# themattinthehatt/behavenet

Measured on AMD Instinct MI355X. Metric: AE training frames/sec (128x128x1, batch 256), higher is better.
Workload: dtype f32; 1 GPU; configs[1]: conv AE default arch, 1x128x128 f32 frames resident in HBM, 12 latents, batch 256 (chunks 200+56), fwd+bwd+Adam(amsgrad)

## Files before the change

### behavenet_amd/_hip.py

```python

import ctypes
import os

import torch

_LIB_NAME = 'libbehavenet_hip.so'
_LIB_PATH = os.environ.get('BN_HIP_LIB') or os.path.join(
    os.path.dirname(os.path.abspath(__file__)), _LIB_NAME)
_lib = None

ACT_NONE, ACT_LRELU, ACT_SIGMOID = 0, 1, 2

PROF_NONE, PROF_CONV_FWD, PROF_CONV_BWD_D, PROF_CONV_BWD_W = 0, 1, 2, 3
PROF_CONVT_FWD, PROF_CONVT_BWD_D, PROF_CONVT_BWD_W, PROF_ADAM = 4, 5, 6, 7
PROF_LINEAR_FWD, PROF_LINEAR_BWD = 8, 9

_c_int, _c_float, _c_size_t, _c_void_p = ctypes.c_int, ctypes.c_float, ctypes.c_size_t, ctypes.c_void_p

_CONV_GEOM = [_c_int] * 12
_ACT_WS = [_c_int, _c_float, _c_void_p, _c_size_t, _c_void_p]

OP_CONV_FWD, OP_CONV_BWD_D, OP_CONV_BWD_W = 1, 2, 3
OP_CONVT_FWD, OP_CONVT_BWD_D, OP_CONVT_BWD_W = 4, 5, 6

# ... 41 lines not shown
    'bn_conv2d_pool2_act_ok': (_c_int, _CONV_GEOM),
    'bn_conv2d_pool2_bwd_weight_ws_bytes': (_c_size_t, _CONV_GEOM),
    'bn_conv2d_pool2_bwd_weight': (
        _c_int, [_c_void_p] * 6 + _CONV_GEOM + [_c_int, _c_float, _c_int, _c_void_p, _c_size_t, _c_void_p]),
    'bn_maxpool2d_act_bwd': (_c_int, [_c_void_p] * 4 + [_c_int] * 4 + [ctypes.c_float, _c_void_p]),
    'bn_maxunpool2d_fwd': (_c_int, [_c_void_p] * 3 + [_c_int] * 3 + [_c_void_p]),
    'bn_maxunpool2d_fwd_k2': (_c_int, [_c_void_p] * 3 + [_c_int] * 3 + [_c_void_p]),
    'bn_maxunpool2d_bwd': (_c_int, [_c_void_p] * 3 + [_c_int] * 3 + [_c_void_p]),
    'bn_act_fwd': (_c_int, [_c_void_p] * 2 + [_c_size_t, _c_int, _c_float, _c_void_p]),
    'bn_act_bwd': (_c_int, [_c_void_p] * 3 + [_c_size_t, _c_int, _c_float, _c_void_p]),
    'bn_linear_ws_bytes': (_c_size_t, [_c_int] * 3),
    'bn_linear_fwd': (_c_int, [_c_void_p] * 4 + [_c_int] * 3 + [_c_void_p, _c_size_t, _c_void_p]),
    'bn_linear_bwd': (
        _c_int, [_c_void_p] * 5 + [_c_int, _c_float, _c_void_p, _c_void_p, _c_int] +
        [_c_int] * 3 + [_c_void_p, _c_size_t, _c_void_p]),
    'bn_sqerr_frame_sums': (_c_int, [_c_void_p] * 4 + [_c_int, _c_size_t, _c_void_p]),
    'bn_sqerr_bwd': (_c_int, [_c_void_p] * 4 + [_c_size_t, _c_float, _c_void_p, _c_void_p]),
    'bn_convT2d_fwd_sqerr_parts': (_c_int, _CONV_GEOM),
    'bn_convT2d_fwd_sqerr_ws_bytes': (_c_size_t, _CONV_GEOM + [_c_int]),
    'bn_convT2d_fwd_sqerr': (
        _c_int, [_c_void_p] * 8 + _CONV_GEOM + [_c_int, _c_float, _c_void_p, _c_size_t, _c_void_p]),
    'bn_scale_frames': (_c_int, [_c_void_p] * 4 + [_c_int, _c_size_t, _c_void_p]),
    'bn_reduce_sum': (_c_int, [_c_void_p] * 2 + [_c_size_t, _c_float, _c_void_p]),
    'bn_reparam_fwd': (_c_int, [_c_void_p] * 4 + [_c_size_t, _c_void_p]),
    'bn_kl_rows': (_c_int, [_c_void_p] * 3 + [_c_int, _c_int, _c_void_p]),
    'bn_reparam_bwd': (_c_int, [_c_void_p] * 4 + [_c_size_t, _c_void_p]),
    'bn_kl_bwd': (_c_int, [_c_void_p] * 4 + [_c_size_t, _c_float, _c_void_p, _c_void_p]),
    'bn_decomposed_kl_fwd': (_c_int, [_c_void_p] * 7 + [_c_int, _c_int, _c_void_p]),
    'bn_decomposed_kl_bwd': (_c_int, [_c_void_p] * 9 + [_c_int, _c_int, _c_void_p]),
    'bn_psvae_head_fwd': (_c_int, [_c_void_p] * 14 + [_c_int] * 3 + [_c_void_p]),
    'bn_psvae_head_combine': (
        _c_int, [_c_void_p] * 4 + [_c_int] + [_c_float] * 3 + [_c_int] + [_c_void_p] * 3),
    'bn_psvae_head_bwd': (
        _c_int, [_c_void_p] * 3 + [_c_int] + [_c_void_p] * 10 + [_c_float] + [_c_void_p] * 5 +
        [_c_int] * 4 + [_c_void_p]),
    'bn_adam_amsgrad_step': (
        _c_int, [_c_void_p] * 5 + [_c_size_t] + [_c_float] * 5 + [_c_int, _c_void_p]),
    'bn_conv2d_first_bf16_ok': (_c_int, _CONV_GEOM),
    'bn_conv2d_bf16_ok': (_c_int, _CONV_GEOM),
    'bn_conv_pack_w_bf16_bytes': (_c_size_t, [_c_int] * 4),
    'bn_conv_pack_w_bf16': (_c_int, [_c_void_p] * 2 + [_c_int] * 4 + [_c_void_p]),
    'bn_conv2d_first_bf16': (
        _c_int, [_c_void_p, _c_int] + [_c_void_p] * 3 + _CONV_GEOM + [_c_int, _c_float, _c_void_p]),
    'bn_conv2d_fwd_bf16': (
        _c_int, [_c_void_p] * 4 + [_c_int] + _CONV_GEOM + [_c_int, _c_float, _c_void_p]),
    'bn_convT2d_bf16_ok': (_c_int, _CONV_GEOM),
# ... 663 lines not shown
        _ptr(dpre, 'dpre'), _ptr(part, 'part'), *geom, act, slope, ws, nbytes, _stream()),
        'bn_convT2d_fwd_sqerr')
    return xhat, dpre, part


def scale_frames(t, frame_scale, group_scale=None, group_of_frame=None):
    N = t.shape[0]
    _check(load().bn_scale_frames(
        _ptr(t, 't'), _ptr(frame_scale, 'frame_scale'),
        _ptr(group_scale, 'group_scale', allow_none=True),
        _ptr(group_of_frame, 'group_of_frame', dtype=torch.int32, allow_none=True),
        N, t.numel() // N, _stream()), 'bn_scale_frames')
    return t


def reduce_sum(t, scale=1.0, out=None):
    if out is None:
        out = torch.empty((), dtype=torch.float32, device=t.device)
    _check(load().bn_reduce_sum(_ptr(t, 'in'), _ptr(out, 'out'), t.numel(), float(scale),
                                _stream()), 'bn_reduce_sum')
    return out


def reparam_fwd(mu, logvar, eps):
    z = torch.empty_like(mu)
    _check(load().bn_reparam_fwd(
        _ptr(mu, 'mu'), _ptr(logvar, 'logvar'), _ptr(eps, 'eps'), _ptr(z, 'z'), mu.numel(),
        _stream()), 'bn_reparam_fwd')
    return z


def kl_rows(mu, logvar):
    N, D = mu.shape
    out = torch.empty((N,), dtype=torch.float32, device=mu.device)
    _check(load().bn_kl_rows(_ptr(mu, 'mu'), _ptr(logvar, 'logvar'), _ptr(out, 'kl_rows'), N, D,
                             _stream()), 'bn_kl_rows')
    return out


DECOMPOSED_KL_MAX_D = 64


def _check_dkl_width(D):
    if D > DECOMPOSED_KL_MAX_D:
        raise ValueError('decomposed KL: %d latent dimensions, the kernels serve at most %d'
                         % (D, DECOMPOSED_KL_MAX_D))
# ... 233 lines not shown
```

### behavenet_amd/csrc/bn_launch.h

```cpp
#pragma once
#include "bn_common.h"

struct GemmArgs {
    const float* A; long sai, sak;
    const float* B; long sbk, sbj;
    float* C; long sci, scj;
    int M, N, K;
    const float* bias_j;
    const float* dact_src;
    int dact; float slope;
    int accumulate;
    float* part;
    int kslice;
};

int bn_launch_down_generic(const float* big, const float* w, const float* bias, float* out,
                           const float* dact_src, const BnGeom& g, int act, int dact, float slope,
                           hipStream_t st);
int bn_launch_up_generic(const float* small, const float* w, const float* bias, float* out,
                         const float* dact_src, const BnGeom& g, int act, int dact, float slope,
                         hipStream_t st);
int bn_launch_wgrad_generic(const float* small, const float* big, float* dw, const BnGeom& g,
                            int accumulate, hipStream_t st);
size_t bn_channel_sum_ws_bytes(int N, int C, int npix);
int bn_launch_channel_sum(const float* t, float* db, int N, int C, int npix, int accumulate,
                          void* ws, size_t ws_bytes, hipStream_t st);

int bn_launch_gemm(const GemmArgs& a, hipStream_t st, void* ws = nullptr, size_t ws_bytes = 0);
size_t bn_gemm_ws_bytes(int M, int N, int K);
int bn_launch_col_sum(const float* dy, float* db, int M, int N, int accumulate, hipStream_t st);
int bn_launch_linear_jobs(const GemmArgs* g0, const GemmArgs* g1, const float* dy, float* db, int M,
                          int N, int accumulate, void* ws, size_t ws_bytes, hipStream_t st);
size_t bn_linear_jobs_ws_bytes(int M, int N, int K);

int bn_launch_act_fwd(const float* x, float* y, size_t n, int act, float slope, hipStream_t st);
int bn_launch_act_bwd(const float* dy, const float* y, float* dpre, size_t n, int act, float slope,
                      hipStream_t st);
int bn_launch_sqerr_frame_sums(const float* pred, const float* target, const float* mask,
                               float* frame_sums, int N, size_t D, hipStream_t st);
int bn_launch_sqerr_bwd(const float* pred, const float* target, const float* mask, float* dpred,
                        size_t n, float scale, const float* gscale, hipStream_t st);
int bn_launch_scale_frames(float* t, const float* frame_scale, const float* group_scale,
                           const int* group_of_frame, int N, size_t D, hipStream_t st);
int bn_launch_reduce_sum(const float* in, float* out, size_t n, float scale, hipStream_t st);
int bn_launch_reparam_fwd(const float* mu, const float* logvar, const float* eps, float* z,
                          size_t n, hipStream_t st);
int bn_launch_kl_rows(const float* mu, const float* logvar, float* kl_rows, int N, int D,
                      hipStream_t st);
int bn_launch_reparam_bwd(const float* dz, const float* z, const float* mu, float* dlogvar,
                          size_t n, hipStream_t st);
int bn_launch_kl_bwd(const float* mu, const float* logvar, float* dmu, float* dlogvar, size_t n,
                     float scale, const float* gscale, hipStream_t st);
int bn_launch_adam(float* p, const float* g, float* m, float* v, float* vmax, size_t n, float lr,
                   float b1, float b2, float eps, float wd, int step, hipStream_t st);
int bn_launch_u8_to_unit_float(const unsigned char* in, float* out, size_t n, hipStream_t st);

bool bn_frame_sq_err_ok(int N, size_t D);
size_t bn_frame_sq_err_ws_bytes_impl(int N, size_t D);
int bn_launch_frame_sq_err(const float* xhat, const void* target, int target_is_u8, const float* mask, float* out,
                           int N, size_t D, float scale, void* ws, hipStream_t st);
int bn_launch_frame_err_finish(const float* part, float* out, int N, unsigned P, float scale, hipStream_t st);

bool bn_unit_float_to_u8_ok(size_t n);
int bn_launch_unit_float_to_u8(const float* in, unsigned char* out, size_t n, hipStream_t st);

size_t bn_batchnorm_ws_bytes_impl(int N, int C);
int bn_launch_bn_stats(const float* x, float* mean, float* var, int N, int C, int HW, void* ws,
// ... 114 lines not shown
```

### behavenet_amd/csrc/capi.hip

```cpp
#include <math.h>
#include <stdio.h>
#include <stdlib.h>
#include <string.h>
#include <hip/hip_ext.h>
#include "bn_common.h"
#include "bn_launch.h"
#include "bn_fast.h"

namespace {
struct ProfState {
    int family = BN_PROF_NONE;
    int C = 0, K = 0;
    static const int kMaxSlots = 2048;
    hipEvent_t ev[4 * kMaxSlots];
    bool taken[kMaxSlots], bracketed[kMaxSlots];
    int created = 0;
    int used = 0;
    double total_ms = 0.0, main_ms = 0.0;
    long launches = 0, main_launches = 0;
    bool bracket = true;
    int nth = -1, seen = 0;
    char kernel_name[96] = "";
} g_prof;

// ... 1554 lines not shown
    if (rc) return rc;
    rc = bn_launch_sqerr_frame_sums(xh, target, mask, part, N, (size_t)Co * Ho * Wo, st);
    if (rc) return rc;
    rc = bn_launch_sqerr_bwd(xh, target, mask, dpre, n_out, 1.f, nullptr, st);
    if (rc) return rc;
    if (act != BN_ACT_NONE) rc = bn_launch_act_bwd(dpre, xh, dpre, n_out, act, slope, st);
    return rc;
}

extern "C" int bn_scale_frames(float* t, const float* frame_scale, const float* group_scale,
                               const int* group_of_frame, int N, size_t D, bn_stream_t stream) {
    if (!t || !frame_scale || N <= 0 || D == 0) return BN_E_BADARG;
    if ((group_scale == nullptr) != (group_of_frame == nullptr)) return BN_E_BADARG;
    return bn_launch_scale_frames(t, frame_scale, group_scale, group_of_frame, N, D,
                                  (hipStream_t)stream);
}

extern "C" int bn_reduce_sum(const float* in, float* out, size_t n, float scale,
                             bn_stream_t stream) {
    if (!in || !out) return BN_E_BADARG;
    return bn_launch_reduce_sum(in, out, n, scale, (hipStream_t)stream);
}

extern "C" int bn_reparam_fwd(const float* mu, const float* logvar, const float* eps, float* z,
                              size_t n, bn_stream_t stream) {
    if (!mu || !logvar || !eps || !z) return BN_E_BADARG;
    if (n == 0) return 0;
    return bn_launch_reparam_fwd(mu, logvar, eps, z, n, (hipStream_t)stream);
}

extern "C" int bn_kl_rows(const float* mu, const float* logvar, float* kl_rows, int N, int D,
                          bn_stream_t stream) {
    if (!mu || !logvar || !kl_rows || N <= 0 || D <= 0) return BN_E_BADARG;
    return bn_launch_kl_rows(mu, logvar, kl_rows, N, D, (hipStream_t)stream);
}

extern "C" int bn_reparam_bwd(const float* dz, const float* z, const float* mu, float* dlogvar,
                              size_t n, bn_stream_t stream) {
    if (!dz || !z || !mu || !dlogvar) return BN_E_BADARG;
    if (n == 0) return 0;
    return bn_launch_reparam_bwd(dz, z, mu, dlogvar, n, (hipStream_t)stream);
}

extern "C" int bn_kl_bwd(const float* mu, const float* logvar, float* dmu, float* dlogvar,
                         size_t n, float scale, const float* gscale, bn_stream_t stream) {
    if (!mu || !logvar || !dmu || !dlogvar) return BN_E_BADARG;
// ... 200 lines not shown
```

### behavenet_amd/csrc/elementwise.hip

```cpp
#include "bn_common.h"
#include "bn_launch.h"

#define EW_THREADS 256
#define EW_MAX_BLOCKS 2048

static inline int ew_blocks(size_t nvec) {
    size_t b = (nvec + EW_THREADS - 1) / EW_THREADS;
    if (b < 1) b = 1;
    if (b > EW_MAX_BLOCKS) b = EW_MAX_BLOCKS;
    return (int)b;
}

static inline bool aligned16(const void* p) { return (((uintptr_t)p) & 15u) == 0; }

__global__ __launch_bounds__(EW_THREADS) void k_act_bwd(
    const float* __restrict__ dy, const float* __restrict__ y, float* __restrict__ dpre, size_t n,
    int vec, int act, float slope) {
    const size_t tid = (size_t)blockIdx.x * EW_THREADS + threadIdx.x;
    const size_t nthreads = (size_t)gridDim.x * EW_THREADS;
    if (vec) {
        const size_t n4 = n >> 2;
        const float4* dy4 = reinterpret_cast<const float4*>(dy);
        const float4* y4 = reinterpret_cast<const float4*>(y);
        float4* o4 = reinterpret_cast<float4*>(dpre);
// ... 71 lines not shown
            if (mask) { const float4 k = m4[i]; o.x *= k.x; o.y *= k.y; o.z *= k.z; o.w *= k.w; }
            o4[i] = o;
        }
        for (size_t i = (n4 << 2) + tid; i < n; i += nthreads) {
            float o = sc * (pred[i] - target[i]); if (mask) o *= mask[i]; dpred[i] = o;
        }
    } else {
        for (size_t i = tid; i < n; i += nthreads) {
            float o = sc * (pred[i] - target[i]); if (mask) o *= mask[i]; dpred[i] = o;
        }
    }
}

__global__ __launch_bounds__(EW_THREADS) void k_reduce_sum(
    const float* __restrict__ in, float* __restrict__ out, size_t n, float scale) {
    __shared__ float red[EW_THREADS / BN_WAVE];
    float acc = 0.f;
    for (size_t i = threadIdx.x; i < n; i += EW_THREADS) acc += in[i];
#pragma unroll
    for (int off = 32; off > 0; off >>= 1) acc += __shfl_down(acc, off, 64);
    if ((threadIdx.x & 63) == 0) red[threadIdx.x >> 6] = acc;
    __syncthreads();
    if (threadIdx.x == 0) out[0] = ((red[0] + red[1]) + (red[2] + red[3])) * scale;
}

__global__ __launch_bounds__(EW_THREADS) void k_reparam_fwd(
    const float* __restrict__ mu, const float* __restrict__ logvar, const float* __restrict__ eps,
    float* __restrict__ z, size_t n) {
    const size_t nthreads = (size_t)gridDim.x * EW_THREADS;
    for (size_t i = (size_t)blockIdx.x * EW_THREADS + threadIdx.x; i < n; i += nthreads)
        z[i] = fmaf(eps[i], expf(logvar[i]), mu[i]);
}

__global__ __launch_bounds__(EW_THREADS) void k_kl_rows(
    const float* __restrict__ mu, const float* __restrict__ logvar, float* __restrict__ kl_rows,
    int N, int D) {
    const int row = blockIdx.x * (EW_THREADS / BN_WAVE) + (threadIdx.x >> 6);
    if (row >= N) return;
    const int lane = threadIdx.x & 63;
    float acc = 0.f;
    for (int d = lane; d < D; d += BN_WAVE) {
        const float lv = logvar[(size_t)row * D + d], m = mu[(size_t)row * D + d];
        acc += expf(lv) - lv + m * m - 1.f;
    }
#pragma unroll
    for (int off = 32; off > 0; off >>= 1) acc += __shfl_down(acc, off, 64);
// ... 152 lines not shown
    } else {
        for (size_t i = tid; i < D; i += nthreads) row[i] *= sc;
    }
}

int bn_launch_scale_frames(float* t, const float* frame_scale, const float* group_scale,
                           const int* group_of_frame, int N, size_t D, hipStream_t st) {
    const int vec = aligned16(t) && (D % 4 == 0);
    const size_t per = vec ? D / 4 : D;
    int bx = (int)((per + EW_THREADS - 1) / EW_THREADS);
    if (bx > 64) bx = 64;
    hipLaunchKernelGGL(k_scale_frames, dim3(bx, N), dim3(EW_THREADS), 0, st, t, frame_scale,
                       group_scale, group_of_frame, D, vec);
    BN_LAUNCH_CHECK();
    return 0;
}

int bn_launch_reduce_sum(const float* in, float* out, size_t n, float scale, hipStream_t st) {
    hipLaunchKernelGGL(k_reduce_sum, dim3(1), dim3(EW_THREADS), 0, st, in, out, n, scale);
    BN_LAUNCH_CHECK();
    return 0;
}

int bn_launch_reparam_fwd(const float* mu, const float* logvar, const float* eps, float* z,
                          size_t n, hipStream_t st) {
    hipLaunchKernelGGL(k_reparam_fwd, dim3(ew_blocks(n)), dim3(EW_THREADS), 0, st, mu, logvar, eps,
                       z, n);
    BN_LAUNCH_CHECK();
    return 0;
}

int bn_launch_kl_rows(const float* mu, const float* logvar, float* kl_rows, int N, int D,
                      hipStream_t st) {
    const int rows_per_block = EW_THREADS / BN_WAVE;
    hipLaunchKernelGGL(k_kl_rows, dim3((N + rows_per_block - 1) / rows_per_block),
                       dim3(EW_THREADS), 0, st, mu, logvar, kl_rows, N, D);
    BN_LAUNCH_CHECK();
    return 0;
}

int bn_launch_reparam_bwd(const float* dz, const float* z, const float* mu, float* dlogvar,
                          size_t n, hipStream_t st) {
    hipLaunchKernelGGL(k_reparam_bwd, dim3(ew_blocks(n)), dim3(EW_THREADS), 0, st, dz, z, mu,
                       dlogvar, n);
    BN_LAUNCH_CHECK();
    return 0;
// ... 32 lines not shown
```

### behavenet_amd/hip_functions.py

```python

import collections.abc
import contextlib
import os
import threading
import warnings

import torch

from behavenet_amd import _hip

LRELU_SLOPE = 0.05

_direct_grads = False


class accumulate_into_param_grads(object):

    def __enter__(self):
        global _direct_grads
        self._prev = _direct_grads
        _direct_grads = True

    def __exit__(self, *exc):
        global _direct_grads
# ... 373 lines not shown
                    rec[i].append((acts[i + 1] > 0).cpu())
        ctx.plan = plan
        ctx.taps = taps
        ctx.need_dx = x.requires_grad
        ctx.param_refs = params
        _note_use(params, any(ctx.needs_input_grad[3:]))
        ctx.save_for_backward(*acts, *params[0::2])
        return h

    @staticmethod
    def backward(ctx, dout):
        plan = ctx.plan
        dout = dout.contiguous()
        top = plan[-1]
        if top.act != _hip.ACT_NONE:
            dpre = _hip.act_bwd(dout, ctx.saved_tensors[len(plan)], top.act, LRELU_SLOPE)
        else:
            dpre = dout
        dx, grads = _stack_backward(ctx, dpre, first_param=3)
        return (None, dx, None) + tuple(grads)


_DGRAD_FIRST = os.environ.get('BN_DGRAD_FIRST', '0') == '1'


def _stack_backward(ctx, dpre, first_param):
    plan = ctx.plan
    n_layers = len(plan)
    saved = ctx.saved_tensors
    acts, weights = saved[:n_layers + 1], saved[n_layers + 1:2 * n_layers + 1]
    n = dpre.shape[0]
    grads = [None] * (2 * n_layers)
    taps = getattr(ctx, 'taps', None)
    tail = []
    for i in range(n_layers - 1, -1, -1):
        layer = plan[i]
        g = layer.geom(n)
        w = weights[i]
        x_in = acts[i]
        if x_in.dtype == torch.uint8:
            x_in = _hip.u8_to_unit_float(x_in) \
                if ctx.needs_input_grad[first_param + 2 * i] else None
        need_w = ctx.needs_input_grad[first_param + 2 * i]
        need_b = ctx.needs_input_grad[first_param + 1 + 2 * i]
        dpre_below = None
        if i > 0 and min(plan[i - 1].cin, plan[i - 1].cout) <= 4 and _DGRAD_FIRST:
            dact_src, dact = acts[i], plan[i - 1].act
            bwd_data = _hip.conv2d_bwd_data if layer.kind == 'conv' else _hip.convT2d_bwd_data
            dpre_below = bwd_data(dpre, w, g, dact_src, dact, LRELU_SLOPE, w5=taps[i] if taps else None)
        if need_w:
            gw = _grad_buffer(ctx.param_refs[2 * i])
            gb = _grad_buffer(ctx.param_refs[2 * i + 1]) if need_b else None
            direct = gw is not None and (gb is not None or not need_b)
            if direct:
                dw, db = gw, gb
            else:
                dw = torch.empty_like(w)
                db = torch.empty((layer.cout,), dtype=w.dtype, device=w.device) if need_b \
                    else None
            wgrad = _hip.conv2d_bwd_weight if layer.kind == 'conv' else _hip.convT2d_bwd_weight
            side = _side_stream(w.device) if (direct and _use_side_stream) else None
            if side is not None and not ctx.need_dx and i < _tail_on_main:
                tail.append(((wgrad, x_in, dpre, dw, db, g), ctx.param_refs[2 * i:2 * i + 2]))
            elif side is not None:
                main = torch.cuda.current_stream(w.device)
                ev = torch.cuda.Event()
                ev.record(main)
# ... 251 lines not shown
    @staticmethod
    def forward(ctx, plan, x, target, mask, bounds, scales, want_xhat, *params):
        if plan[-1].kind != 'convT':
            raise ValueError('the fused pixel loss follows a transposed convolution')
        x = x.contiguous()
        target = target.contiguous()
        mask = mask.contiguous() if mask is not None else None
        acts = [x]
        h = x
        taps = _stack_taps(plan, x.shape[0], params) if x.is_cuda else None
        for i, layer in enumerate(plan[:-1]):
            h = _fwd(layer, h, params[2 * i].detach(), params[2 * i + 1].detach(), w5=taps[i] if taps else None)
            acts.append(h)
        top = plan[-1]
        n = h.shape[0]
        xhat, dpre, part = _hip.convT2d_fwd_sqerr(
            h, params[-2].detach(), params[-1].detach(), target, mask, top.geom(n), top.act,
            LRELU_SLOPE, bool(want_xhat))
        if _sign_tap is not None:
            rec = _sign_tap.setdefault(id(plan), [[] for _ in plan])
            for i, layer in enumerate(plan[:-1]):
                if layer.act == _hip.ACT_LRELU:
                    rec[i].append((acts[i + 1] > 0).cpu())
        out = torch.empty((len(bounds),), dtype=torch.float32, device=x.device)
        for c, ((beg, end), sc) in enumerate(zip(bounds, scales)):
            _hip.reduce_sum(part[beg:end], float(sc), out=out[c:c + 1])
        ctx.plan = plan
        ctx.taps = taps
        ctx.need_dx = x.requires_grad
        ctx.param_refs = params
        ctx.bounds, ctx.scales = list(bounds), [float(sc) for sc in scales]
        ctx.consumed = False
        _note_use(params, any(ctx.needs_input_grad[7:]))
        ctx.save_for_backward(*acts, dpre, *params[0::2])
        if xhat is not None:
            ctx.mark_non_differentiable(xhat)
        return out, xhat

    @staticmethod
    def backward(ctx, g, _g_xhat):
        if ctx.consumed:
            raise RuntimeError('ConvStackSqErrFn: backward twice (dL/dpre is scaled in place)')
        ctx.consumed = True
        n_layers = len(ctx.plan)
        dpre = ctx.saved_tensors[n_layers]
        fs, ci = _frame_scales(dpre.shape[0], ctx.bounds, ctx.scales, dpre.device)
        _hip.scale_frames(dpre, fs, g.contiguous(), ci)
        dx, grads = _stack_backward(ctx, dpre, first_param=7)
        return (None, dx, None, None, None, None, None) + tuple(grads)


def conv_stack_sq_err(plan, x, params, target, mask, bounds, scales, want_xhat=False):
    return ConvStackSqErrFn.apply(plan, x, target, mask, tuple(bounds), tuple(scales),
                                  bool(want_xhat), *params)


class FusedPixelLoss(object):

    def __init__(self, x_hat, chunk_terms, kind, bounds):
        self.x_hat = x_hat
        self.chunk_terms = chunk_terms
        self.kind = kind
        self.bounds = list(bounds)


_DEVICE_CONSTANTS = {}


def device_constant(values, device):
    key = (tuple(float(v) for v in values), str(device))
    t = _DEVICE_CONSTANTS.get(key)
# ... 267 lines not shown
        a, b, mask = ctx.saved_tensors
        g = g.contiguous()
        da = db = None
        if ctx.needs_input_grad[0]:
            da = _hip.sqerr_bwd(a, b, mask, ctx.scale, g)
        if ctx.needs_input_grad[1]:
            db = _hip.sqerr_bwd(b, a, mask, ctx.scale, g)
        return da, db, None, None


def sq_err(a, b, mask, scale):
    return SqErrFn.apply(a, b, mask, scale)


class ChunkedSqErrFn(torch.autograd.Function):

    @staticmethod
    def forward(ctx, a, b, mask, bounds, scales):
        a, b = a.contiguous(), b.contiguous()
        mask = mask.contiguous() if mask is not None else None
        ctx.save_for_backward(a, b, mask)
        ctx.bounds, ctx.scales = list(bounds), [float(s) for s in scales]
        sums = _hip.sqerr_frame_sums(a, b, mask)
        out = torch.empty((len(ctx.bounds),), dtype=torch.float32, device=a.device)
        for i, ((beg, end), s) in enumerate(zip(ctx.bounds, ctx.scales)):
            _hip.reduce_sum(sums[beg:end], s, out=out[i:i + 1])
        return out

    @staticmethod
    def backward(ctx, g):
        a, b, mask = ctx.saved_tensors
        g = g.contiguous()
        grads = []
        for need, p, t in ((ctx.needs_input_grad[0], a, b), (ctx.needs_input_grad[1], b, a)):
            if not need:
                grads.append(None)
                continue
            d = torch.empty_like(p)
            for i, ((beg, end), s) in enumerate(zip(ctx.bounds, ctx.scales)):
                _hip.sqerr_bwd(p[beg:end], t[beg:end], mask[beg:end] if mask is not None else None,
                               s, g[i:i + 1], out=d[beg:end])
            grads.append(d)
        return grads[0], grads[1], None, None, None


def chunked_sq_err(a, b, mask, bounds, scales):
    return ChunkedSqErrFn.apply(a, b, mask, bounds, scales)


class ReparamFn(torch.autograd.Function):
# ... 429 lines not shown
```

### include/behavenet_hip.h

```cpp
#ifndef BEHAVENET_HIP_H
#define BEHAVENET_HIP_H

#include <stddef.h>

#ifdef __cplusplus
extern "C" {
#endif

#define BN_E_BADARG   (-1)
#define BN_E_SHAPE    (-2)
#define BN_E_WORKSPACE (-3)

#define BN_ACT_NONE    0
#define BN_ACT_LRELU   1
#define BN_ACT_SIGMOID 2

typedef void* bn_stream_t;

int         bn_version(void);
const char* bn_build_arch(void);
const char* bn_error_string(int code);

#define BN_OP_CONV_FWD    1
#define BN_OP_CONV_BWD_D  2
// ... 99 lines not shown
                        void* ws, size_t ws_bytes, bn_stream_t stream);
int bn_batchnorm_bwd_reduce(const float* x, const float* y, const float* dy, const float* mean,
                            const float* invstd, float* sum_dz, float* sum_dzx, int N, int C,
                            int HW, int act, float slope, void* ws, size_t ws_bytes,
                            bn_stream_t stream);
int bn_batchnorm_bwd_apply(const float* x, const float* y, const float* dy, const float* mean,
                           const float* invstd, const float* gamma, const float* sum_dz,
                           const float* sum_dzx, float* dx, int N, int C, int HW, float inv_count,
                           int act, float slope, bn_stream_t stream);

size_t bn_linear_ws_bytes(int M, int K, int N);
int bn_linear_fwd(const float* x, const float* w, const float* b, float* y,
                  int M, int K, int N, void* ws, size_t ws_bytes, bn_stream_t stream);
int bn_linear_bwd(const float* x, const float* w, const float* dy,
                  float* dx, const float* dact_src, int dact, float slope,
                  float* dw, float* db, int accumulate,
                  int M, int K, int N, void* ws, size_t ws_bytes, bn_stream_t stream);

int bn_sqerr_frame_sums(const float* pred, const float* target, const float* mask,
                        float* frame_sums, int N, size_t D, bn_stream_t stream);
int bn_sqerr_bwd(const float* pred, const float* target, const float* mask, float* dpred,
                 size_t n, float scale, const float* gscale, bn_stream_t stream);
int bn_reduce_sum(const float* in, float* out, size_t n, float scale, bn_stream_t stream);

int bn_reparam_fwd(const float* mu, const float* logvar, const float* eps, float* z,
                   size_t n, bn_stream_t stream);
int bn_kl_rows(const float* mu, const float* logvar, float* kl_rows, int N, int D,
               bn_stream_t stream);
int bn_reparam_bwd(const float* dz, const float* z, const float* mu, float* dlogvar, size_t n,
                   bn_stream_t stream);
int bn_kl_bwd(const float* mu, const float* logvar, float* dmu, float* dlogvar, size_t n,
              float scale, const float* gscale, bn_stream_t stream);

int bn_decomposed_kl_fwd(const float* z, const float* mu, const float* logvar, float* out3,
                         float* log_qz, float* lse, float* terms, int N, int D,
                         bn_stream_t stream);
int bn_decomposed_kl_bwd(const float* z, const float* mu, const float* logvar,
                         const float* log_qz, const float* lse, const float* g3, float* dz,
                         float* dmu, float* dlogvar, int N, int D, bn_stream_t stream);

int bn_psvae_head_fwd(const float* y, const float* w, const float* logvar, const float* eps,
                      const float* Dw, const float* Db, const float* labels, const float* lmask,
                      float* z, float* z_u, float* lv_u, float* yhat, float* row_sq,
                      float* row_kl, int N, int L, int U, bn_stream_t stream);
int bn_psvae_head_combine(const float* row_sq, const float* row_kl, const float* dkl3,
                          const int* bounds, int n_chunks, float alpha, float kl, float beta,
                          int L, float* T, float* cols5, bn_stream_t stream);
int bn_psvae_head_bwd(const float* dz, const float* gT, const int* bounds, int n_chunks,
                      const float* y, const float* logvar, const float* eps, const float* yhat,
                      const float* labels, const float* lmask, const float* Dw, const float* gz_u,
                      const float* gmu_u, const float* glv_u, float alpha, float* dy, float* dw,
                      float* dlogvar, float* dDw, float* dDb, int accumulate, int N, int L, int U,
                      bn_stream_t stream);

int bn_convT2d_fwd_sqerr_parts(int N, int Ci, int Hi, int Wi, int Co, int R, int S, int stride,
                               int crop_t, int crop_l, int Ho, int Wo);
size_t bn_convT2d_fwd_sqerr_ws_bytes(int N, int Ci, int Hi, int Wi, int Co, int R, int S,
                                     int stride, int crop_t, int crop_l, int Ho, int Wo,
                                     int with_xhat);
int bn_convT2d_fwd_sqerr(const float* x, const float* w, const float* b, const float* target,
                         const float* mask, float* xhat, float* dpre, float* part,
                         int N, int Ci, int Hi, int Wi, int Co, int R, int S, int stride,
                         int crop_t, int crop_l, int Ho, int Wo, int act, float slope,
                         void* ws, size_t ws_bytes, bn_stream_t stream);
int bn_scale_frames(float* t, const float* frame_scale, const float* group_scale,
                    const int* group_of_frame, int N, size_t D, bn_stream_t stream);

int bn_adam_amsgrad_step(float* p, const float* g, float* m, float* v, float* vmax, size_t n,
                         float lr, float beta1, float beta2, float eps, float weight_decay,
                         int step, bn_stream_t stream);

size_t bn_conv2d_fwd_u8_ws_bytes(int N, int C, int H, int W, int K, int R, int S, int stride,
                                 int pad_t, int pad_l, int P, int Q, int act);
int bn_conv2d_fwd_u8(const unsigned char* x, const float* w, const float* b, float* y,
                     int N, int C, int H, int W, int K, int R, int S, int stride,
                     int pad_t, int pad_l, int P, int Q, int act, float slope,
                     void* ws, size_t ws_bytes, bn_stream_t stream);

int bn_conv2d_first_bf16_ok(int N, int C, int H, int W, int K, int R, int S, int stride,
                            int pad_t, int pad_l, int P, int Q);
int bn_conv2d_bf16_ok(int N, int C, int H, int W, int K, int R, int S, int stride,
                      int pad_t, int pad_l, int P, int Q);
size_t bn_conv_pack_w_bf16_bytes(int K, int C, int R, int S);
int bn_conv_pack_w_bf16(const float* w, void* wp, int K, int C, int R, int S, bn_stream_t stream);
int bn_conv2d_first_bf16(const void* x, int x_is_u8, const float* w, const float* b, void* y,
                         int N, int C, int H, int W, int K, int R, int S, int stride,
                         int pad_t, int pad_l, int P, int Q, int act, float slope, bn_stream_t stream);
int bn_conv2d_fwd_bf16(const void* x, const void* wp, const float* b, void* y, int out_f32,
                       int N, int C, int H, int W, int K, int R, int S, int stride,
// ... 60 lines not shown
```

Before: 59020 frames/s.

## Fuse top convT backward (frame scaling, dgrad, wgrad, bias) into one MFMA kernel

Adds a persistent MFMA kernel for the last transposed-conv layer (Co=1, 5x5, stride 2) backward. In one pass it applies per-frame loss scaling, computes the input gradient with the leaky-ReLU mask, and accumulates the weight and bias gradients, with double-buffered LDS DMA prefetch and a separate reduction of per-unit partials. This avoids a separate scale_frames pass and separate dgrad/wgrad/bias kernels that each re-read the full-resolution gradient. It also batches the per-chunk loss reductions into a single grouped-reduce launch, which cuts launch count, at the cost of a large specialised kernel that only covers certain geometries.

Result: no change. 59510 frames/s (median of 6 runs) (+0.8%).

```diff
diff --git a/behavenet_amd/_hip.py b/behavenet_amd/_hip.py
--- a/behavenet_amd/_hip.py
+++ b/behavenet_amd/_hip.py
@@ -87,6 +87,11 @@
         _c_int, [_c_void_p] * 8 + _CONV_GEOM + [_c_int, _c_float, _c_void_p, _c_size_t, _c_void_p]),
     'bn_scale_frames': (_c_int, [_c_void_p] * 4 + [_c_int, _c_size_t, _c_void_p]),
     'bn_reduce_sum': (_c_int, [_c_void_p] * 2 + [_c_size_t, _c_float, _c_void_p]),
+    'bn_reduce_sum_groups': (_c_int, [_c_void_p] * 5 + [_c_int, _c_void_p]),
+    'bn_convT2d_bwd_top_c1_ok': (_c_int, _CONV_GEOM + [_c_int]),
+    'bn_convT2d_bwd_top_c1_ws_bytes': (_c_size_t, _CONV_GEOM),
+    'bn_convT2d_bwd_top_c1': (
+        _c_int, [_c_void_p] * 9 + _CONV_GEOM + [_c_int, _c_float, _c_int, _c_void_p, _c_size_t, _c_void_p]),
     'bn_reparam_fwd': (_c_int, [_c_void_p] * 4 + [_c_size_t, _c_void_p]),
     'bn_kl_rows': (_c_int, [_c_void_p] * 3 + [_c_int, _c_int, _c_void_p]),
     'bn_reparam_bwd': (_c_int, [_c_void_p] * 4 + [_c_size_t, _c_void_p]),
@@ -796,6 +801,39 @@
     return out
 
 
+def reduce_sum_groups(t, bounds, scales, out=None):
+    n = len(bounds)
+    if out is None:
+        out = torch.empty((n,), dtype=torch.float32, device=t.device)
+    row = t.numel() // t.shape[0] if t.shape[0] else 0
+    begins = (ctypes.c_longlong * n)(*[int(b) * row for b, _ in bounds])
+    lengths = (ctypes.c_longlong * n)(*[(int(e) - int(b)) * row for b, e in bounds])
+    sc = (ctypes.c_float * n)(*[float(s) for s in scales])
+    _check(load().bn_reduce_sum_groups(_ptr(t, 'in'), _ptr(out, 'out'), begins, lengths, sc, n, _stream()),
+           'bn_reduce_sum_groups')
+    return out
+
+
+def convT2d_bwd_top_c1_ok(geom, dact):
+    return bool(load().bn_convT2d_bwd_top_c1_ok(*[int(v) for v in geom], int(dact)))
+
+
+def convT2d_bwd_top_c1(a, dpre, w, frame_scale, group_scale, group_of_frame, dw, db, geom, dact, slope,
+                       accumulate):
+    N, Ci, Hi, Wi = geom[:4]
+    lib = load()
+    dz = torch.empty((N, Ci, Hi, Wi), dtype=torch.float32, device=a.device)
+    nbytes = lib.bn_convT2d_bwd_top_c1_ws_bytes(*geom)
+    ws = _arena(a.device, nbytes, 'top_bwd') if nbytes else None
+    _check(lib.bn_convT2d_bwd_top_c1(
+        _ptr(a, 'a'), _ptr(dpre, 'dpre'), _ptr(w, 'w'), _ptr(frame_scale, 'frame_scale'),
+        _ptr(group_scale, 'group_scale', allow_none=True),
+        _ptr(group_of_frame, 'group_of_frame', dtype=torch.int32, allow_none=True),
+        _ptr(dz, 'dz'), _ptr(dw, 'dw'), _ptr(db, 'db'), *geom, int(dact), float(slope), int(accumulate),
+        ws, nbytes, _stream()), 'bn_convT2d_bwd_top_c1')
+    return dz
+
+
 def reparam_fwd(mu, logvar, eps):
     z = torch.empty_like(mu)
     _check(load().bn_reparam_fwd(
diff --git a/behavenet_amd/csrc/bn_launch.h b/behavenet_amd/csrc/bn_launch.h
--- a/behavenet_amd/csrc/bn_launch.h
+++ b/behavenet_amd/csrc/bn_launch.h
@@ -43,6 +43,8 @@
 int bn_launch_scale_frames(float* t, const float* frame_scale, const float* group_scale,
                            const int* group_of_frame, int N, size_t D, hipStream_t st);
 int bn_launch_reduce_sum(const float* in, float* out, size_t n, float scale, hipStream_t st);
+int bn_launch_reduce_sum_groups(const float* in, float* out, const long long* begins, const long long* lengths,
+                                const float* scales, int n_groups, hipStream_t st);
 int bn_launch_reparam_fwd(const float* mu, const float* logvar, const float* eps, float* z,
                           size_t n, hipStream_t st);
 int bn_launch_kl_rows(const float* mu, const float* logvar, float* kl_rows, int N, int D,
diff --git a/behavenet_amd/csrc/capi.hip b/behavenet_amd/csrc/capi.hip
--- a/behavenet_amd/csrc/capi.hip
+++ b/behavenet_amd/csrc/capi.hip
@@ -1600,6 +1600,15 @@
     return bn_launch_reduce_sum(in, out, n, scale, (hipStream_t)stream);
 }
 
+extern "C" int bn_reduce_sum_groups(const float* in, float* out, const long long* begins,
+                                    const long long* lengths, const float* scales, int n_groups,
+                                    bn_stream_t stream) {
+    if (!in || !out || !begins || !lengths || !scales || n_groups <= 0) return BN_E_BADARG;
+    for (int c = 0; c < n_groups; ++c)
+        if (begins[c] < 0 || lengths[c] <= 0) return BN_E_BADARG;
+    return bn_launch_reduce_sum_groups(in, out, begins, lengths, scales, n_groups, (hipStream_t)stream);
+}
+
 extern "C" int bn_reparam_fwd(const float* mu, const float* logvar, const float* eps, float* z,
                               size_t n, bn_stream_t stream) {
     if (!mu || !logvar || !eps || !z) return BN_E_BADARG;
diff --git a/behavenet_amd/csrc/conv_top_bwd.hip b/behavenet_amd/csrc/conv_top_bwd.hip
--- /dev/null
+++ b/behavenet_amd/csrc/conv_top_bwd.hip
@@ -0,0 +1,399 @@
+#include <hip/hip_ext.h>
+#include "bn_common.h"
+
+typedef float tb_f16 __attribute__((ext_vector_type(16)));
+typedef float tb_f4 __attribute__((ext_vector_type(4)));
+
+#define TB_THREADS 256
+#define TB_OOB 0x7fffffff
+#define TB_SP 260
+#define TB_SPU 8
+#define TB_ZL 16
+
+template <int TW> struct TbGeo {
+    static constexpr int TR = 256 / TW;
+    static constexpr int IH = 2 * TR + 3;
+    static constexpr int RW = 2 * TW + 8;
+    static constexpr int NGR = RW / 4;
+    static constexpr int NG = IH * NGR;
+    static constexpr int PATCH = NG * 4;
+};
+template <int TW, int CG> struct TbLds {
+    static constexpr int TILE = 32 * CG * TB_SP;
+    static constexpr int BUF = TILE + TbGeo<TW>::PATCH;
+    static constexpr int BYTES = 2 * BUF * 4;
+};
+
+struct TbArgs {
+    const float* a;
+    const float* dpre;
+    float* dz;
+    float* part;
+    float* bpart;
+    int N, Hs, Ws, Hb, Wb, pt, pl;
+    int has_mask;
+    float slope;
+    int n_stages, n_units, spf, ncb;
+};
+
+__device__ __forceinline__ void tb_barrier() { asm volatile("s_waitcnt lgkmcnt(0)\n s_barrier" ::: "memory"); }
+__device__ __forceinline__ void tb_dma16(__amdgpu_buffer_rsrc_t rsrc, float* lds, int voffset, int soffset) {
+    __builtin_amdgcn_raw_ptr_buffer_load_lds(rsrc, lds, 16, voffset, soffset, 0, 0);
+}
+
+template <int TW, int CG>
+__global__ __launch_bounds__(TB_THREADS) void k_top_bwd_c1(
+    const float* __restrict__ w,
+    const float* __restrict__ fs,
+    const float* __restrict__ gs,
+    const int* __restrict__ gof,
+    const TbArgs p) {
+    typedef TbGeo<TW> G;
+    typedef TbLds<TW, CG> L;
+    constexpr int C = 32 * CG, TR = G::TR, RW = G::RW, NGR = G::NGR, NG = G::NG;
+    constexpr int NDMA = 8 * CG;
+    static_assert(NG <= 2 * TB_THREADS, "two patch groups per thread");
+    static_assert(4 * CG * 16 * 64 + 4 <= L::TILE, "reduction scratch inside one `a` tile");
+    extern __shared__ __attribute__((aligned(16))) float tsm[];
+    const int tid = threadIdx.x, lane = tid & 63;
+    const int wv = __builtin_amdgcn_readfirstlane(tid >> 6);
+    const int li = lane & 31, kk = lane >> 5;
+    const int PQ = p.Hs * p.Ws;
+
+    const __amdgpu_buffer_rsrc_t ra = __builtin_amdgcn_make_buffer_rsrc(
+        (void*)p.a, 0, (int)((size_t)p.N * C * PQ * 4), 0x00020000);
+    const __amdgpu_buffer_rsrc_t rd = __builtin_amdgcn_make_buffer_rsrc(
+        (void*)p.dpre, 0, (int)((size_t)p.N * p.Hb * p.Wb * 4), 0x00020000);
+    const __amdgpu_buffer_rsrc_t ro = __builtin_amdgcn_make_buffer_rsrc(
+        (void*)p.dz, 0, (int)((size_t)p.N * C * PQ * 4), 0x00020000);
+
+    const int svo = ((lane / (TW / 4)) * p.Ws + 4 * (lane % (TW / 4))) * 4;
+    int pg_y[2], pg_j[2], pg_off[2];
+    bool pg_own[2];
+#pragma unroll
+    for (int k = 0; k < 2; ++k) {
+        const int e = tid + TB_THREADS * k;
+        const int y = e / NGR, j = e - y * NGR;
+        pg_y[k] = e < NG ? y : -0x10000;
+        pg_j[k] = j;
+        pg_off[k] = (y * p.Wb + 4 * j) * 4;
+        pg_own[k] = e < NG && j >= 1 && j <= NGR - 2 && y >= p.pt && y < p.pt + 2 * TR;
+    }
+    float wr[CG][13];
+#pragma unroll
+    for (int g = 0; g < CG; ++g)
+#pragma unroll
+        for (int t = 0; t < 13; ++t) {
+            const int tap = 2 * t + kk;
+            wr[g][t] = tap < 25 ? w[(32 * g + li) * 25 + tap] : 0.f;
+        }
+    const int a_col = 4 - p.pl + 2 * li;
+    const int kkA = kk, kkB = kk * (RW - 4);
+    const int st_lane = (4 * kk * PQ + li) * 4;
+    const int tap = li < 25 ? li : 0;
+    const int tr = tap / 5, ts = tap - tr * 5;
+    const int wq_a = li * TB_SP + kk;
+    const int wq_b = tr * RW + 4 - p.pl + ts + 2 * kk;
+
+    tb_f16 wacc[CG][2];
+#pragma unroll
+    for (int g = 0; g < CG; ++g)
+#pragma unroll
+        for (int h = 0; h < 2; ++h)
+#pragma unroll
+            for (int e = 0; e < 16; ++e) wacc[g][h][e] = 0.f;
+    float bsum = 0.f;
+
+    tb_f4 pr[2];
+    float sc_next = 0.f;
+    auto decode = [&](int st, int& n, int& p0, int& q0) {
+        n = st / p.spf;
+        const int rem = st - n * p.spf;
+        const int rb = rem / p.ncb;
+        p0 = rb * TR;
+        q0 = (rem - rb * p.ncb) * TW;
+    };
+    auto issue_patch = [&](int st, bool live) {
+        int n, p0, q0;
+        decode(st, n, p0, q0);
+        float sc = fs[n];
+        if (gs) sc *= gs[gof[n]];
+        sc_next = sc;
+        const int hb0 = 2 * p0 - p.pt, wb0 = 2 * q0 - 4;
+        const int base = ((n * p.Hb + hb0) * p.Wb + wb0) * 4;
+#pragma unroll
+        for (int k = 0; k < 2; ++k) {
+            const int hb = hb0 + pg_y[k], wb = wb0 + 4 * pg_j[k];
+            const bool ok = live && hb >= 0 && hb < p.Hb && wb >= 0 && wb < p.Wb;
+            pr[k] = __builtin_bit_cast(tb_f4, __builtin_amdgcn_raw_buffer_load_b128(
+                rd, ok ? base + pg_off[k] : TB_OOB, 0, 0));
+        }
+    };
+    const int dma_step = 4 * PQ * 4;
+    int dma_so = 0, dma_vo = svo;
+    auto plan_dma = [&](int st, bool live) {
+        int n, p0, q0;
+        decode(st, n, p0, q0);
+        dma_so = (((n * C + wv) * p.Hs + p0) * p.Ws + q0) * 4;
+        dma_vo = live ? svo : TB_OOB;
+    };
+    auto issue_dma = [&](const int d, const int buf) __attribute__((always_inline)) {
+        tb_dma16(ra, tsm + buf * L::BUF + (wv + 4 * d) * TB_SP, dma_vo, dma_so + d * dma_step);
+    };
+
+    const int Gw = gridDim.x;
+    int u = blockIdx.x;
+    int st = u * TB_SPU;
+    int uend = st + TB_SPU < p.n_stages ? st + TB_SPU : p.n_stages;
+    plan_dma(st, true);
+#pragma unroll
+    for (int d = 0; d < NDMA; ++d) issue_dma(d, 0);
+    issue_patch(st, true);
+    auto write_patch = [&](int buf) {
+        float* patch = tsm + buf * L::BUF + L::TILE;
+        const float sc = sc_next;
+#pragma unroll
+        for (int k = 0; k < 2; ++k) {
+            if (pg_y[k] < 0) continue;
+            tb_f4 v = pr[k];
+            v.x *= sc; v.y *= sc; v.z *= sc; v.w *= sc;
+            *reinterpret_cast<tb_f4*>(patch + 4 * (tid + TB_THREADS * k)) = v;
+            if (pg_own[k]) bsum += (v.x + v.y) + (v.z + v.w);
+        }
+    };
+    asm volatile("s_waitcnt vmcnt(0)" ::: "memory");
+    write_patch(0);
+    int cur = 0;
+#pragma unroll 1
+    for (;;) {
+        float* tile = tsm + cur * L::BUF;
+        float* patch = tile + L::TILE;
+        tb_barrier();
+
+        int nst = st + 1, nu = u, nend = uend;
+        bool more = true;
+        if (nst >= uend) {
+            nu = u + Gw;
+            if (nu < p.n_units) {
+                nst = nu * TB_SPU;
+                nend = nst + TB_SPU < p.n_stages ? nst + TB_SPU : p.n_stages;
+            } else {
+                more = false;
+            }
+        }
+        issue_patch(more ? nst : st, more);
+        plan_dma(more ? nst : st, more);
+
+        int n, p0, q0;
+        decode(st, n, p0, q0);
+#pragma unroll
+        for (int j = 0; j < 2; ++j) {
+            const int row = TW == 64 ? wv : wv + 4 * j;
+            const int col0 = TW == 64 ? 32 * j : 0;
+            const float* ar = patch + (2 * row) * RW + a_col + 2 * col0;
+            const float* arA = ar + kkA;
+            const float* arB = ar + kkB;
+            const float* mrow = tile + (4 * kk) * TB_SP + row * TW + col0 + li;
+#pragma unroll
+            for (int g = 0; g < CG; ++g) {
+                tb_f16 acc;
+#pragma unroll
+                for (int e = 0; e < 16; ++e) acc[e] = 0.f;
+#pragma unroll
+                for (int t = 0; t < 13; ++t) {
+                    const int t0 = ((2 * t) / 5) * RW + (2 * t) % 5;
+                    const float* at = ((2 * t) % 5 == 4 && t != 12) ? arB : arA;
+                    acc = __builtin_amdgcn_mfma_f32_32x32x2f32(wr[g][t], at[t0], acc, 0, 0, 0);
+                    if (j == 0 && t < 8) issue_dma(g * 8 + t, cur ^ 1);
+                }
+                float d[16];
+#pragma unroll
+                for (int e = 0; e < 16; ++e)
+                    d[e] = mrow[(32 * g + (e & 3) + 8 * (e >> 2)) * TB_SP];
+                const int so0 = (((n * C + 32 * g) * p.Hs + p0 + row) * p.Ws + q0 + col0) * 4;
+#pragma unroll
+                for (int e = 0; e < 16; ++e) {
+                    const int chb = (e & 3) + 8 * (e >> 2);
+                    float v = acc[e];
+                    if (p.has_mask) v *= d[e] > 0.f ? 1.f : p.slope;
+                    __builtin_amdgcn_raw_buffer_store_b32(__builtin_bit_cast(int, v), ro, st_lane,
+                                                          so0 + chb * PQ * 4, 0);
+                }
+            }
+        }
+#pragma unroll
+        for (int j = 0; j < 2; ++j) {
+            const int row = TW == 64 ? wv : wv + 4 * j;
+            const int col0 = TW == 64 ? 32 * j : 0;
+            const float* aq = tile + wq_a + row * TW + col0;
+            const float* bq = patch + wq_b + 2 * row * RW + 2 * col0;
+#pragma unroll
+            for (int t = 0; t < 16; ++t) {
+                const float bv = bq[4 * t];
+#pragma unroll
+                for (int g = 0; g < CG; ++g)
+                    wacc[g][t & 1] = __builtin_amdgcn_mfma_f32_32x32x2f32(aq[32 * g * TB_SP + 2 * t], bv,
+                                                                        wacc[g][t & 1], 0, 0, 0);
+            }
+        }
+
+        if (st + 1 >= uend) {
+            tb_barrier();
+            float* red = tile;
+#pragma unroll
+            for (int g = 0; g < CG; ++g)
+#pragma unroll
+                for (int e = 0; e < 16; ++e) {
+                    red[((wv * CG + g) * 16 + e) * 64 + lane] = wacc[g][0][e] + wacc[g][1][e];
+                    wacc[g][0][e] = 0.f;
+                    wacc[g][1][e] = 0.f;
+                }
+            float bs = bsum;
+#pragma unroll
+            for (int off = 32; off > 0; off >>= 1) bs += __shfl_down(bs, off, 64);
+            if (lane == 0) red[4 * CG * 16 * 64 + wv] = bs;
+            bsum = 0.f;
+            tb_barrier();
+            if (wv == 0 && li < 25) {
+#pragma unroll
+                for (int g = 0; g < CG; ++g)
+#pragma unroll
+                    for (int e = 0; e < 16; ++e) {
+                        const int s = (g * 16 + e) * 64 + lane;
+                        const float v = (red[s] + red[s + CG * 16 * 64]) +
+                                        (red[s + 2 * CG * 16 * 64] + red[s + 3 * CG * 16 * 64]);
+                        const int ch = 32 * g + (e & 3) + 8 * (e >> 2) + 4 * kk;
+                        p.part[(size_t)u * (C * 25) + ch * 25 + li] = v;
+                    }
+            }
+            if (tid == 0) {
+                const float* rb = red + 4 * CG * 16 * 64;
+                p.bpart[u] = (rb[0] + rb[1]) + (rb[2] + rb[3]);
+            }
+        }
+        if (!more) break;
+        asm volatile("s_waitcnt vmcnt(%0)" :: "n"(16 * (CG + 1)) : "memory");
+        write_patch(cur ^ 1);
+        st = nst; u = nu; uend = nend;
+        cur ^= 1;
+    }
+}
+
+__global__ __launch_bounds__(64 * TB_ZL) void k_top_bwd_sum(const float* __restrict__ part,
+                                                            const float* __restrict__ bpart, float* __restrict__ dw,
+                                                            float* __restrict__ db, int total, int units,
+                                                            int accumulate) {
+    __shared__ float red[TB_ZL][64];
+    const int il = threadIdx.x & 63, zl = threadIdx.x >> 6;
+    const int i = blockIdx.x * 64 + il;
+    const bool is_b = i == total;
+    const float* src = is_b ? bpart : part + i;
+    const size_t stride = is_b ? 1 : (size_t)total;
+    float s0 = 0.f, s1 = 0.f, s2 = 0.f, s3 = 0.f;
+    if (i <= total) {
+        int z = zl;
+        for (; z + 3 * TB_ZL < units; z += 4 * TB_ZL) {
+            s0 += src[(size_t)z * stride];
+            s1 += src[(size_t)(z + TB_ZL) * stride];
+            s2 += src[(size_t)(z + 2 * TB_ZL) * stride];
+            s3 += src[(size_t)(z + 3 * TB_ZL) * stride];
+        }
+        for (; z < units; z += TB_ZL) s0 += src[(size_t)z * stride];
+    }
+    red[zl][il] = (s0 + s1) + (s2 + s3);
+    __syncthreads();
+    if (zl == 0 && i <= total) {
+        float v = 0.f;
+#pragma unroll
+        for (int k = 0; k < TB_ZL; k += 4)
+            v += (red[k][il] + red[k + 1][il]) + (red[k + 2][il] + red[k + 3][il]);
+        float* o = is_b ? db : dw + i;
+        if (o) *o = accumulate ? *o + v : v;
+    }
+}
+
+struct TbPlan { bool ok; int tw, cg, n_stages, n_units, spf, ncb; size_t ws_bytes; };
+
+static TbPlan tb_plan(int N, int Ci, int Hi, int Wi, int Co, int R, int S, int stride, int crop_t, int crop_l,
+                      int Ho, int Wo, int dact) {
+    TbPlan pl = {false, 0, 0, 0, 0, 0, 0, 0};
+    if (N <= 0 || Hi <= 0 || Wi <= 0) return pl;
+    if (Co != 1 || R != 5 || S != 5 || stride != 2) return pl;
+    if (Ci != 32 && Ci != 64) return pl;
+    if ((Wi % 32) != 0 || (Hi % 8) != 0 || Ho != 2 * Hi || Wo != 2 * Wi) return pl;
+    if (crop_t < 0 || crop_t > 2 || crop_l < 0 || crop_l > 2) return pl;
+    if (dact != BN_ACT_NONE && dact != BN_ACT_LRELU) return pl;
+    if ((size_t)N * Ci * Hi * Wi * 4 >= 0x7fffffffull) return pl;
+    pl.tw = (Wi % 64) == 0 ? 64 : 32;
+    pl.cg = Ci / 32;
+    pl.ncb = Wi / pl.tw;
+    pl.spf = (Hi / (256 / pl.tw)) * pl.ncb;
+    if ((size_t)N * pl.spf >= 0x7fffffffull / TB_SPU) return pl;
+    pl.n_stages = N * pl.spf;
+    pl.n_units = (pl.n_stages + TB_SPU - 1) / TB_SPU;
+    pl.ws_bytes = ((size_t)pl.n_units * (Ci * 25) + (size_t)pl.n_units) * sizeof(float);
+    pl.ok = true;
+    return pl;
+}
+
+extern "C" int bn_convT2d_bwd_top_c1_ok(int N, int Ci, int Hi, int Wi, int Co, int R, int S, int stride,
+                                        int crop_t, int crop_l, int Ho, int Wo, int dact) {
+    return tb_plan(N, Ci, Hi, Wi, Co, R, S, stride, crop_t, crop_l, Ho, Wo, dact).ok ? 1 : 0;
+}
+
+extern "C" size_t bn_convT2d_bwd_top_c1_ws_bytes(int N, int Ci, int Hi, int Wi, int Co, int R, int S, int stride,
+                                                 int crop_t, int crop_l, int Ho, int Wo) {
+    return tb_plan(N, Ci, Hi, Wi, Co, R, S, stride, crop_t, crop_l, Ho, Wo, BN_ACT_NONE).ws_bytes;
+}
+
+template <int TW, int CG>
+static int tb_launch(const float* w, const float* fs, const float* gs, const int* gof, const TbArgs& a, int grid,
+                     hipStream_t st) {
+    typedef TbLds<TW, CG> L;
+    static bool attr_set = false;
+    if (!attr_set) {
+        const hipError_t e = hipFuncSetAttribute((const void*)k_top_bwd_c1<TW, CG>,
+                                                 hipFuncAttributeMaxDynamicSharedMemorySize, L::BYTES);
+        if (e != hipSuccess) return (int)e;
+        attr_set = true;
+    }
+    BN_LAUNCH_MAIN((k_top_bwd_c1<TW, CG>), dim3(grid), dim3(TB_THREADS), L::BYTES, st, w, fs, gs, gof, a);
+    BN_LAUNCH_CHECK();
+    return 0;
+}
+
+extern "C" int bn_convT2d_bwd_top_c1(const float* a3, const float* dpre, const float* w, const float* frame_scale,
+                                     const float* group_scale, const int* group_of_frame, float* dz, float* dw,
+                                     float* db, int N, int Ci, int Hi, int Wi, int Co, int R, int S, int stride,
+                                     int crop_t, int crop_l, int Ho, int Wo, int dact, float slope, int accumulate,
+                                     void* ws, size_t ws_bytes, bn_stream_t stream) {
+    if (!a3 || !dpre || !w || !frame_scale || !dz || !dw || !db) return BN_E_BADARG;
+    if ((group_scale == nullptr) != (group_of_frame == nullptr)) return BN_E_BADARG;
+    const TbPlan pl = tb_plan(N, Ci, Hi, Wi, Co, R, S, stride, crop_t, crop_l, Ho, Wo, dact);
+    if (!pl.ok) return BN_E_SHAPE;
+    if (((((uintptr_t)a3) | ((uintptr_t)dpre)) & 15u) != 0) return BN_E_SHAPE;
+    if (!ws || ws_bytes < pl.ws_bytes) return BN_E_WORKSPACE;
+    hipStream_t st = (hipStream_t)stream;
+    TbArgs a;
+    a.a = a3; a.dpre = dpre; a.dz = dz;
+    a.part = (float*)ws;
+    a.bpart = (float*)ws + (size_t)pl.n_units * (Ci * 25);
+    a.N = N; a.Hs = Hi; a.Ws = Wi; a.Hb = Ho; a.Wb = Wo; a.pt = crop_t; a.pl = crop_l;
+    a.has_mask = dact == BN_ACT_LRELU ? 1 : 0;
+    a.slope = slope;
+    a.n_stages = pl.n_stages; a.n_units = pl.n_units; a.spf = pl.spf; a.ncb = pl.ncb;
+    const int cap = pl.cg == 1 ? 512 : 256;
+    const int grid = pl.n_units < cap ? pl.n_units : cap;
+    BnProfScope prof(BN_PROF_CONVT_BWD_D, Co, Ci, "k_top_bwd_c1 + k_top_bwd_sum", st);
+    int rc;
+#define TB_GO(TW, CG) tb_launch<TW, CG>(w, frame_scale, group_scale, group_of_frame, a, grid, st)
+    if (pl.tw == 64) rc = pl.cg == 1 ? TB_GO(64, 1) : TB_GO(64, 2);
+    else             rc = pl.cg == 1 ? TB_GO(32, 1) : TB_GO(32, 2);
+#undef TB_GO
+    if (rc) return rc;
+    const int total = Ci * 25;
+    hipLaunchKernelGGL(k_top_bwd_sum, dim3((total + 1 + 63) / 64), dim3(64 * TB_ZL), 0, st, a.part, a.bpart, dw, db,
+                       total, pl.n_units, accumulate);
+    BN_LAUNCH_CHECK();
+    return 0;
+}
diff --git a/behavenet_amd/csrc/elementwise.hip b/behavenet_amd/csrc/elementwise.hip
--- a/behavenet_amd/csrc/elementwise.hip
+++ b/behavenet_amd/csrc/elementwise.hip
@@ -117,6 +117,23 @@
     if ((threadIdx.x & 63) == 0) red[threadIdx.x >> 6] = acc;
     __syncthreads();
     if (threadIdx.x == 0) out[0] = ((red[0] + red[1]) + (red[2] + red[3])) * scale;
+}
+
+#define RG_MAX 32
+struct BnReduceGroups { size_t beg[RG_MAX]; size_t len[RG_MAX]; float scale[RG_MAX]; };
+__global__ __launch_bounds__(EW_THREADS) void k_reduce_sum_groups(
+    const float* __restrict__ in_, float* __restrict__ out, BnReduceGroups gr) {
+    __shared__ float red[EW_THREADS / BN_WAVE];
+    const int c = blockIdx.x;
+    const float* in = in_ + gr.beg[c];
+    const size_t n = gr.len[c];
+    float acc = 0.f;
+    for (size_t i = threadIdx.x; i < n; i += EW_THREADS) acc += in[i];
+#pragma unroll
+    for (int off = 32; off > 0; off >>= 1) acc += __shfl_down(acc, off, 64);
+    if ((threadIdx.x & 63) == 0) red[threadIdx.x >> 6] = acc;
+    __syncthreads();
+    if (threadIdx.x == 0) out[c] = ((red[0] + red[1]) + (red[2] + red[3])) * gr.scale[c];
 }
 
 __global__ __launch_bounds__(EW_THREADS) void k_reparam_fwd(
@@ -315,6 +332,22 @@
     return 0;
 }
 
+int bn_launch_reduce_sum_groups(const float* in, float* out, const long long* begins, const long long* lengths,
+                                const float* scales, int n_groups, hipStream_t st) {
+    for (int g0 = 0; g0 < n_groups; g0 += RG_MAX) {
+        const int ng = n_groups - g0 < RG_MAX ? n_groups - g0 : RG_MAX;
+        BnReduceGroups gr;
+        for (int c = 0; c < RG_MAX; ++c) {
+            gr.beg[c] = c < ng ? (size_t)begins[g0 + c] : 0;
+            gr.len[c] = c < ng ? (size_t)lengths[g0 + c] : 0;
+            gr.scale[c] = c < ng ? scales[g0 + c] : 0.f;
+        }
+        hipLaunchKernelGGL(k_reduce_sum_groups, dim3(ng), dim3(EW_THREADS), 0, st, in, out + g0, gr);
+        BN_LAUNCH_CHECK();
+    }
+    return 0;
+}
+
 int bn_launch_reparam_fwd(const float* mu, const float* logvar, const float* eps, float* z,
                           size_t n, hipStream_t st) {
     hipLaunchKernelGGL(k_reparam_fwd, dim3(ew_blocks(n)), dim3(EW_THREADS), 0, st, mu, logvar, eps,
diff --git a/behavenet_amd/hip_functions.py b/behavenet_amd/hip_functions.py
--- a/behavenet_amd/hip_functions.py
+++ b/behavenet_amd/hip_functions.py
@@ -419,9 +419,10 @@
 
 
 _DGRAD_FIRST = os.environ.get('BN_DGRAD_FIRST', '0') == '1'
-
-
-def _stack_backward(ctx, dpre, first_param):
+_FUSED_TOP_BWD = os.environ.get('BN_FUSED_TOP_BWD', '1') != '0'
+
+
+def _stack_backward(ctx, dpre, first_param, top_scale=None):
     plan = ctx.plan
     n_layers = len(plan)
     saved = ctx.saved_tensors
@@ -440,6 +441,20 @@
                 if ctx.needs_input_grad[first_param + 2 * i] else None
         need_w = ctx.needs_input_grad[first_param + 2 * i]
         need_b = ctx.needs_input_grad[first_param + 1 + 2 * i]
+        if i == n_layers - 1 and top_scale is not None:
+            fs, gup, ci = top_scale
+            dact = plan[i - 1].act if i > 0 else _hip.ACT_NONE
+            gw = gb = None
+            if _FUSED_TOP_BWD and need_w and need_b and (i > 0 or ctx.need_dx) and layer.kind == 'convT' \
+                    and x_in is not None and x_in.dtype == torch.float32 \
+                    and _hip.convT2d_bwd_top_c1_ok(g, dact):
+                gw = _grad_buffer(ctx.param_refs[2 * i])
+                gb = _grad_buffer(ctx.param_refs[2 * i + 1])
+            if gw is not None and gb is not None:
+                dpre = _hip.convT2d_bwd_top_c1(x_in, dpre, w, fs, gup, ci, gw, gb, g, dact, LRELU_SLOPE, True)
+                _report_ready(ctx.param_refs[2 * i:2 * i + 2])
+                continue
+            _hip.scale_frames(dpre, fs, gup, ci)
         dpre_below = None
         if i > 0 and min(plan[i - 1].cin, plan[i - 1].cout) <= 4 and _DGRAD_FIRST:
             dact_src, dact = acts[i], plan[i - 1].act
@@ -737,9 +752,7 @@
             for i, layer in enumerate(plan[:-1]):
                 if layer.act == _hip.ACT_LRELU:
                     rec[i].append((acts[i + 1] > 0).cpu())
-        out = torch.empty((len(bounds),), dtype=torch.float32, device=x.device)
-        for c, ((beg, end), sc) in enumerate(zip(bounds, scales)):
-            _hip.reduce_sum(part[beg:end], float(sc), out=out[c:c + 1])
+        out = _hip.reduce_sum_groups(part, bounds, scales)
         ctx.plan = plan
         ctx.taps = taps
         ctx.need_dx = x.requires_grad
@@ -760,8 +773,7 @@
         n_layers = len(ctx.plan)
         dpre = ctx.saved_tensors[n_layers]
         fs, ci = _frame_scales(dpre.shape[0], ctx.bounds, ctx.scales, dpre.device)
-        _hip.scale_frames(dpre, fs, g.contiguous(), ci)
-        dx, grads = _stack_backward(ctx, dpre, first_param=7)
+        dx, grads = _stack_backward(ctx, dpre, first_param=7, top_scale=(fs, g.contiguous(), ci))
         return (None, dx, None, None, None, None, None) + tuple(grads)
 
 
@@ -1075,10 +1087,7 @@
         ctx.save_for_backward(a, b, mask)
         ctx.bounds, ctx.scales = list(bounds), [float(s) for s in scales]
         sums = _hip.sqerr_frame_sums(a, b, mask)
-        out = torch.empty((len(ctx.bounds),), dtype=torch.float32, device=a.device)
-        for i, ((beg, end), s) in enumerate(zip(ctx.bounds, ctx.scales)):
-            _hip.reduce_sum(sums[beg:end], s, out=out[i:i + 1])
-        return out
+        return _hip.reduce_sum_groups(sums, ctx.bounds, ctx.scales)
 
     @staticmethod
     def backward(ctx, g):
diff --git a/include/behavenet_hip.h b/include/behavenet_hip.h
--- a/include/behavenet_hip.h
+++ b/include/behavenet_hip.h
@@ -145,6 +145,8 @@
 int bn_sqerr_bwd(const float* pred, const float* target, const float* mask, float* dpred,
                  size_t n, float scale, const float* gscale, bn_stream_t stream);
 int bn_reduce_sum(const float* in, float* out, size_t n, float scale, bn_stream_t stream);
+int bn_reduce_sum_groups(const float* in, float* out, const long long* begins, const long long* lengths,
+                         const float* scales, int n_groups, bn_stream_t stream);
 
 int bn_reparam_fwd(const float* mu, const float* logvar, const float* eps, float* z,
                    size_t n, bn_stream_t stream);
@@ -188,6 +190,16 @@
                          void* ws, size_t ws_bytes, bn_stream_t stream);
 int bn_scale_frames(float* t, const float* frame_scale, const float* group_scale,
                     const int* group_of_frame, int N, size_t D, bn_stream_t stream);
+
+int bn_convT2d_bwd_top_c1_ok(int N, int Ci, int Hi, int Wi, int Co, int R, int S, int stride,
+                             int crop_t, int crop_l, int Ho, int Wo, int dact);
+size_t bn_convT2d_bwd_top_c1_ws_bytes(int N, int Ci, int Hi, int Wi, int Co, int R, int S, int stride,
+                                      int crop_t, int crop_l, int Ho, int Wo);
+int bn_convT2d_bwd_top_c1(const float* a, const float* dpre, const float* w, const float* frame_scale,
+                          const float* group_scale, const int* group_of_frame, float* dz, float* dw,
+                          float* db, int N, int Ci, int Hi, int Wi, int Co, int R, int S, int stride,
+                          int crop_t, int crop_l, int Ho, int Wo, int dact, float slope, int accumulate,
+                          void* ws, size_t ws_bytes, bn_stream_t stream);
 
 int bn_adam_amsgrad_step(float* p, const float* g, float* m, float* v, float* vmax, size_t n,
                          float lr, float beta1, float beta2, float eps, float weight_decay,
```
